# yynil/RWKVTTS

Hardware: AMD Instinct MI355X
Metric: audio-tokens/sec/GPU (train fwd+bwd) RWKV7-0.4B L=4096; 1->8 GPU scaling (higher is better)
Workload: dtype bf16; 1 GPU; RWKV7-0.4B Spark layout train step (fwd+bwd+AdamW), B=8/GPU L=4096, synthetic text+speech tokens, random init (BASELINE.json configs[1]); global_batch=8, seq_len=4096, parallelism=dp1, grad_allreduce=none

## Files before the change

include/rwkv7_hip.h:

```cpp
#ifndef RWKV7_HIP_H
#define RWKV7_HIP_H

#include <stddef.h>

#ifdef __cplusplus
extern "C" {
#endif

#define RWKV7_OK 0
#define RWKV7_EINVAL (-1)
#define RWKV7_ECHUNK (-2)
#define RWKV7_EHEAD  (-3)
#define RWKV7_ESHAPE (-4)

#define RWKV7_HEAD_SIZE 64
#define RWKV7_CHUNK_LEN 16

typedef void *rwkv7_stream_t;

const char *rwkv7_version(void);

int rwkv7_wkv_fwd_bf16(int B, int T, int H, const void *w, const void *q, const void *k, const void *v,
                       const void *a, const void *b, void *y, float *s, float *sa, rwkv7_stream_t stream);
int rwkv7_wkv_fwd_f32(int B, int T, int H, const void *w, const void *q, const void *k, const void *v,
// ... 184 lines not shown
                                   const float *z, const void *e_vk, void *dw, void *dq, void *dk, void *dv,
                                   void *da, void *db, rwkv7_stream_t stream);
int rwkv7_wkv_chunk_fwd_state_bf16(int B, int T, int H, const void *w, const void *q, const void *k, const void *v,
                                   const void *a, const void *b, const float *tinv, void *y, float *sa, void *hs,
                                   const float *h0, float *hT, rwkv7_stream_t stream);
int rwkv7_wkv_chunk_bseq_state_bf16(int B, int T, int H, const void *w, const void *q, const void *a, const void *b,
                                    const void *dy, const float *tinv, void *e_vk, float *z,
                                    const float *dhT, float *dh0, rwkv7_stream_t stream);
int rwkv7_wkv_chunk_fwd_state_seq_bf16(int B, int T, int H, const void *w, const void *q, const void *k, const void *v,
                                       const void *a, const void *b, const float *tinv, void *y, float *sa, void *hs,
                                       const int *seq_chunk_off, int nseq, const float *h0, float *hT, rwkv7_stream_t stream);
int rwkv7_wkv_chunk_bseq_state_seq_bf16(int B, int T, int H, const void *w, const void *q, const void *a, const void *b,
                                        const void *dy, const float *tinv, void *e_vk, float *z, const int *seq_chunk_off, int nseq,
                                        const float *dhT, float *dh0, rwkv7_stream_t stream);
#define RWKV7_STATE_ROW_ZERO (1 << 30)
int rwkv7_wkv_chunk_fwd_state_rows_bf16(int T, int H, const void *w, const void *q, const void *k, const void *v, const void *a,
                                        const void *b, const float *tinv, void *y, const int *seq_chunk_off, int nseq, float *state,
                                        const int *state_row, rwkv7_stream_t stream);
int rwkv7_add_ln_mix_rows_fwd_bf16(int T, int D, int nmix, const void *x, const void *branch, const void *gamma, const void *beta,
                                   float eps, const void *mask, const void *params, const int *prev_src, const int *last_dst,
                                   const void *x_prev_rd, void *x_prev, void *x_out, void *out, int nblocks, int run_len,
                                   rwkv7_stream_t stream);
int rwkv7_cache_rows_commit_bf16(int layers, int n, const void *const *src_tbl, void *const *dst_tbl, const int *src_row,
                                 const int *dst_row, int D, int H, rwkv7_stream_t stream);
#define RWKV7_SEED_ZERO (-1)
int rwkv7_cache_rows_seed_bf16(int layers, int n, const void *const *src_tbl, void *const *dst_tbl, const int *src_row,
                               const int *dst_row, int D, int H, rwkv7_stream_t stream);
int rwkv7_cache_rows_retain_bf16(int layers, int slots, const void *const *src_tbl, void *const *dst_tbl, const unsigned char *live,
                                 unsigned char *armed, const int *retain_row, int *ticket, int D, int H, rwkv7_stream_t stream);
int rwkv7_state_rows_expand_f32(int layers, int n, const void *const *master_tbl, void *const *dst_tbl, const int *voice, int D, int H,
                                rwkv7_stream_t stream);
int rwkv7_state_rows_adamw_f32(int layers, int n, int A, const void *const *grad_tbl, void *const *master_tbl, void *const *m_tbl,
                               void *const *v_tbl, void *const *store_tbl, const int *seg_start, const int *seg_rows, const int *seg_info,
                               const float *skip_flag, float lr, float beta1, float beta2, float eps, float weight_decay,
                               float grad_scale, int D, int H, rwkv7_stream_t stream);
int rwkv7_ce_fwd_bwd_bf16(long rows, int V, void *logits, const long *labels, long ignore_index, float scale, float *loss_rows,
                          rwkv7_stream_t stream);
int rwkv7_ce_fwd_bwd_ls_bf16(long rows, int V, void *logits, const long *labels, long ignore_index, float scale, float *loss_rows,
                             float label_smoothing, rwkv7_stream_t stream);
int rwkv7_ce_fwd_bwd_ld_bf16(long rows, int V, long ld, void *logits, const long *labels, long ignore_index, float scale, float *loss_rows,
                             float label_smoothing, rwkv7_stream_t stream);
int rwkv7_ce_reg_fwd_bwd_bf16(long rows, int V, long ld, void *logits, const long *labels, long ignore_index, float scale, float *loss_rows,
                              float label_smoothing, float z_coef, float max_coef, float *lse_rows, float *max_rows,
                              rwkv7_stream_t stream);
int rwkv7_ce_seq_bwd_bf16(long rows, int V, long ld, void *logits, const long *labels, long ignore_index, long row0, long n_seq,
                          const long *seq_start, const float *seq_scale, float *loss_rows, rwkv7_stream_t stream);
int rwkv7_ce_policy_fwd_bwd_bf16(long rows, int V, long ld, void *logits, const long *labels, long ignore_index, long row0, long n_seq,
                                 const long *seq_start, const float *adv, const float *seq_w, const float *old_lp, const float *ref_lp,
                                 float eps_lo, float eps_hi, float beta, float *lp_rows, float *loss_rows, float *kl_rows,
                                 float *clip_rows, rwkv7_stream_t stream);
int rwkv7_kl_acc_fwd_bwd_bf16(long rows, int V, long ld, const void *logits, void *dlogits, const long *labels, long ignore_index,
                              float smoothing, float scale, float *loss_rows, int *correct_rows, rwkv7_stream_t stream);
int rwkv7_head_eval_bf16(long rows, int V, long ld, const void *logits, const long *labels, long ignore_index, int kind, float smoothing,
                         float *loss_rows, int *correct_rows, int *argmax_rows, rwkv7_stream_t stream);
int rwkv7_seq_scores_f32(long n_seq, const long *seq_start, const float *loss_rows, const int *correct_rows, const long *labels,
                         long ignore_index, double *loss_sum, long *tokens, long *correct, float *worst_loss, long *worst_row,
                         rwkv7_stream_t stream);

int rwkv7_adamw_bf16(long n, float *p32, const void *g16, float *m, float *v, void *p16, float lr, float beta1, float beta2,
                     float eps, float weight_decay, int step, rwkv7_stream_t stream);
int rwkv7_adamw_groups_bf16(long n, float *p32, const void *g16, float *m, float *v, void *p16, const unsigned char *slab_group,
                            const float *group_tab, int ngroups, const float *skip_flag, float lr, float beta1, float beta2,
                            float eps, int step, rwkv7_stream_t stream);
int rwkv7_adamw_groups_clip_bf16(long n, float *p32, const void *g16, float *m, float *v, void *p16, const unsigned char *slab_group,
                                 const float *group_tab, int ngroups, const float *skip_flag, const float *sumsq, float max_norm,
                                 float lr, float beta1, float beta2, float eps, int step, rwkv7_stream_t stream);

long rwkv7_grad_sumsq_workspace_bytes(long n);
int rwkv7_grad_sumsq_bf16(long n, const void *g16, float *partials, float *out, int accumulate, rwkv7_stream_t stream);
int rwkv7_grad_accum_bf16(long n, float *acc32, const void *g16, int first, rwkv7_stream_t stream);
int rwkv7_grad_fold_bf16(long n, const float *acc32, void *g16, float inv_count, rwkv7_stream_t stream);

long rwkv7_buf_digest_workspace_bytes(long n_words);
int rwkv7_buf_digest_u32(long n_words, long first_index, const void *buf, unsigned long long *partials, unsigned long long *out,
                         int accumulate, rwkv7_stream_t stream);
int rwkv7_buf_snapshot_digest_u32(long n_words, long first_index, const void *src, void *dst, unsigned long long *partials,
                                  unsigned long long *out, int accumulate, rwkv7_stream_t stream);

int rwkv7_sum_slabs_bf16(long n, int S, const float *parts, void *out, int accumulate, rwkv7_stream_t stream);
int rwkv7_transpose_bf16(int R, int C, const void *in, void *out, rwkv7_stream_t stream);
int rwkv7_gather_rows_bf16(long n_out, int D, const void *src, const int *idx, void *out, rwkv7_stream_t stream);
int rwkv7_wgrad_skinny_bf16(long M, int N, int K, int S, const void *dy, const void *x, float *parts, rwkv7_stream_t stream);
int rwkv7_wgrad_mid_bf16(long M, int N, int K, int S, const void *dy, const void *x, float *parts, rwkv7_stream_t stream);

int rwkv7_gemm_nt_bf16(int M, int N, int K, const void *A, const void *W, void *C, int epilogue, rwkv7_stream_t stream);
int rwkv7_gemm_nt_relusq_bwd_bf16(int M, int N, int K, const void *A, const void *W, const void *aux, void *C, rwkv7_stream_t stream);
int rwkv7_gemm_nt_relusq_bwd_s_bf16(int M, int N, int K, const void *A, const void *W, const void *s, void *C, rwkv7_stream_t stream);
int rwkv7_gemm_nt_add_bf16(int M, int N, int K, const void *A, const void *W, const void *resid, void *C, rwkv7_stream_t stream);

int rwkv7_mix_lora_wcat_fwd_bf16(int nb, const int *ranks, const void *const *w1, const void *const *mu, int D, void *wcat,
                                 rwkv7_stream_t stream);
int rwkv7_mix_lora_wcat_bwd_bf16(int nb, const int *ranks, const void *const *w1, const void *const *mu, int D, const void *dwcat,
                                 void *const *dw1, void *const *dmu, rwkv7_stream_t stream);
int rwkv7_mix_lora_combine_fwd_bf16(int nb, const int *ranks, const int *acts, long M, int T, const void *G, const void *mask,
                                    void *const *out, rwkv7_stream_t stream);
int rwkv7_mix_lora_combine_bwd_bf16(int nb, const int *ranks, const int *acts, long M, int T, const void *mask, const void *const *y,
                                    const void *const *dy, void *dG, rwkv7_stream_t stream);

int rwkv7_lora_down_pack_bf16(int nb, const int *ranks, const void *const *w1, int D, void *packed, rwkv7_stream_t stream);
int rwkv7_lora_down_fwd_bf16(int nb, const int *ranks, const int *acts, long M, int T, int D, const void *x, const void *mask,
                             const void *const *mu, const void *packed, void *const *out, rwkv7_stream_t stream);

int rwkv7_gemv32_bf16(int M, int N, int K, const void *x, const void *w, const void *bias, void *y, rwkv7_stream_t stream);

enum {
    RWKV7_DEC_LN0_W, RWKV7_DEC_LN0_B, RWKV7_DEC_LN1_W, RWKV7_DEC_LN1_B, RWKV7_DEC_LN2_W, RWKV7_DEC_LN2_B,
    RWKV7_DEC_XR, RWKV7_DEC_XW, RWKV7_DEC_XK, RWKV7_DEC_XV, RWKV7_DEC_XA, RWKV7_DEC_XG,
    RWKV7_DEC_WR, RWKV7_DEC_WK, RWKV7_DEC_WV, RWKV7_DEC_WO,
    RWKV7_DEC_W1, RWKV7_DEC_W2, RWKV7_DEC_W0, RWKV7_DEC_A1, RWKV7_DEC_A2, RWKV7_DEC_A0,
    RWKV7_DEC_V1, RWKV7_DEC_V2, RWKV7_DEC_V0, RWKV7_DEC_G1, RWKV7_DEC_G2,
    RWKV7_DEC_KK, RWKV7_DEC_KA, RWKV7_DEC_RK, RWKV7_DEC_GNW, RWKV7_DEC_GNB,
    RWKV7_DEC_FXK, RWKV7_DEC_WKEY, RWKV7_DEC_WVAL,
    RWKV7_DEC_ATT_XPREV, RWKV7_DEC_ATT_KV , RWKV7_DEC_FFN_XPREV,
    RWKV7_DEC_COUNT
};
typedef struct rwkv7_decode_dims {
    int B, D, H, L, F, V;
    int Rw, Ra, Rv, Rg;
    float ln_eps, gn_eps;
} rwkv7_decode_dims;
int rwkv7_decode_layer_ptrs(void);
size_t rwkv7_decode_workspace_bytes(const rwkv7_decode_dims *dims);
int rwkv7_decode_step_bf16(const rwkv7_decode_dims *dims, const void *const *layer_tbl, const void *x_in, const void *norm_w,
                           const void *norm_b, const void *head_w, const void *head_b, float *logits, void *workspace,
                           int persistent, rwkv7_stream_t stream);
int rwkv7_decode_step_tbl_bf16(const rwkv7_decode_dims *dims, const void *const *layer_tbl, const void *const *layer_tbl_host,
                               const void *x_in, const void *norm_w, const void *norm_b, const void *head_w, const void *head_b,
                               float *logits, void *workspace, int persistent, rwkv7_stream_t stream);
size_t rwkv7_decode_wide_workspace_bytes(const rwkv7_decode_dims *dims);
int rwkv7_decode_step_wide_bf16(const rwkv7_decode_dims *dims, const void *const *layer_tbl, const void *const *layer_tbl_host,
                                const void *x_in, const void *norm_w, const void *norm_b, const void *head_w, const void *head_b,
                                float *logits, void *workspace, rwkv7_stream_t stream);

int rwkv7_sample_rows_f32(int rows, int nseg, const float *logits, long ld, const int *seg_off, const int *seg_len, const int *allow_lo,
                          const int *allow_hi, const int *suppress, int nsuppress, int max_domain, int do_sample, int top_k, float top_p,
                          float temperature, unsigned long long seed, const long *step, long *out, rwkv7_stream_t stream);
typedef struct rwkv7_sample_tail {
    unsigned char *unfinished;
    long eos, pad;
    long *ids;
    long *seq;
    long seq_ld;
    const void *emb;
    void *x;
    int D;
} rwkv7_sample_tail;
int rwkv7_sample_rows_tail_f32(int rows, const float *logits, long ld, const int *seg_off, const int *seg_len, const int *allow_lo,
                               const int *allow_hi, const int *suppress, int nsuppress, int max_domain, int do_sample, int top_k, float top_p,
                               float temperature, unsigned long long seed, const long *step, long *out, const rwkv7_sample_tail *tail,
                               int min_eos_id, long min_eos_until, rwkv7_stream_t stream);
typedef struct rwkv7_slot_state {
    long *step;
    long *limit;
    long *min_until;
    unsigned long long *seed;
    float *inv_temp;
    int *top_k;
    float *top_p;
    unsigned char *do_sample;
    unsigned char *live;
    long *ids;
    long *seq;
    long seq_ld;
    const void *emb;
    void *x;
    int D;
// ... 105 lines not shown
```

rwkvtts_amd/csrc/capi.hip:

```cpp
#include <hip/hip_runtime.h>
#include <math.h>

#include "../../include/rwkv7_hip.h"
#include "launchers.h"
#include "ln_row.h"

using rwkv7::any_null;

extern "C" {

const char *rwkv7_version(void) { return "rwkv7_hip 0.1.0 gfx950"; }

#define FWD_BODY(IMPL, CW)                                                                   \
    if (B <= 0 || T <= 0 || H <= 0 || any_null({w, q, k, v, a, b, y})) return RWKV7_EINVAL; \
    if ((s == nullptr) != (sa == nullptr)) return RWKV7_EINVAL;                              \
    if (T % RWKV7_CHUNK_LEN != 0) return RWKV7_ECHUNK;                                       \
    if ((CW) != 0 && (CW) != 4 && (CW) != 8) return RWKV7_ESHAPE;                            \
    return rwkv7::IMPL(B, T, H, w, q, k, v, a, b, y, s, sa, nullptr, CW, (hipStream_t)stream);

int rwkv7_wkv_fwd_bf16(int B, int T, int H, const void *w, const void *q, const void *k, const void *v,
                       const void *a, const void *b, void *y, float *s, float *sa, rwkv7_stream_t stream) {
    FWD_BODY(wkv_fwd_bf16, 0)
}
int rwkv7_wkv_fwd_f32(int B, int T, int H, const void *w, const void *q, const void *k, const void *v,
// ... 486 lines not shown
    if (rows <= 0 || V <= 0 || any_null({(const void *)logits, (const void *)labels, (const void *)loss_rows})) return RWKV7_EINVAL;
    if (!(label_smoothing >= 0.f && label_smoothing < 1.f)) return RWKV7_EINVAL;
    return rwkv7::ce_fwd_bwd(rows, V, V, logits, labels, ignore_index, scale, loss_rows, label_smoothing, (hipStream_t)stream);
}
int rwkv7_ce_fwd_bwd_ld_bf16(long rows, int V, long ld, void *logits, const long *labels, long ignore_index, float scale, float *loss_rows,
                             float label_smoothing, rwkv7_stream_t stream) {
    if (rows <= 0 || V <= 0 || ld < V || any_null({(const void *)logits, (const void *)labels, (const void *)loss_rows})) return RWKV7_EINVAL;
    if (!(label_smoothing >= 0.f && label_smoothing < 1.f)) return RWKV7_EINVAL;
    return rwkv7::ce_fwd_bwd(rows, V, ld, logits, labels, ignore_index, scale, loss_rows, label_smoothing, (hipStream_t)stream);
}
int rwkv7_ce_reg_fwd_bwd_bf16(long rows, int V, long ld, void *logits, const long *labels, long ignore_index, float scale, float *loss_rows,
                              float label_smoothing, float z_coef, float max_coef, float *lse_rows, float *max_rows,
                              rwkv7_stream_t stream) {
    if (rows <= 0 || V <= 0 || ld < V || any_null({(const void *)logits, (const void *)labels, (const void *)loss_rows})) return RWKV7_EINVAL;
    if (!(label_smoothing >= 0.f && label_smoothing < 1.f)) return RWKV7_EINVAL;
    if (!(z_coef >= 0.f && z_coef < INFINITY && max_coef >= 0.f && max_coef < INFINITY)) return RWKV7_EINVAL;
    return rwkv7::ce_reg_fwd_bwd(rows, V, ld, logits, labels, ignore_index, scale, loss_rows, label_smoothing, z_coef, max_coef, lse_rows,
                                 max_rows, (hipStream_t)stream);
}
int rwkv7_ce_seq_bwd_bf16(long rows, int V, long ld, void *logits, const long *labels, long ignore_index, long row0, long n_seq,
                          const long *seq_start, const float *seq_scale, float *loss_rows, rwkv7_stream_t stream) {
    if (rows <= 0 || V <= 0 || ld < V || row0 < 0 || n_seq <= 0 ||
        any_null({(const void *)logits, (const void *)labels, (const void *)seq_start, (const void *)seq_scale}))
        return RWKV7_EINVAL;
    return rwkv7::ce_seq_bwd(rows, V, ld, logits, labels, ignore_index, row0, n_seq, seq_start, seq_scale, loss_rows, (hipStream_t)stream);
}
int rwkv7_ce_policy_fwd_bwd_bf16(long rows, int V, long ld, void *logits, const long *labels, long ignore_index, long row0, long n_seq,
                                 const long *seq_start, const float *adv, const float *seq_w, const float *old_lp, const float *ref_lp,
                                 float eps_lo, float eps_hi, float beta, float *lp_rows, float *loss_rows, float *kl_rows,
                                 float *clip_rows, rwkv7_stream_t stream) {
    if (rows <= 0 || V <= 0 || ld < V || row0 < 0 || n_seq <= 0 ||
        any_null({(const void *)logits, (const void *)labels, (const void *)seq_start, (const void *)adv, (const void *)seq_w,
                  (const void *)old_lp}))
        return RWKV7_EINVAL;
    if (!(eps_lo >= 0.f && eps_lo < 1.f && eps_hi >= 0.f)) return RWKV7_EINVAL;
    return rwkv7::ce_policy_fwd_bwd(rows, V, ld, logits, labels, ignore_index, row0, n_seq, seq_start, adv, seq_w, old_lp, ref_lp, eps_lo,
                                    eps_hi, beta, lp_rows, loss_rows, kl_rows, clip_rows, (hipStream_t)stream);
}
static float kl_entropy_const(float smoothing, int V) {
    const double s = (double)smoothing;
    return (float)((1.0 - s) * log(1.0 - s) + (s > 0.0 ? s * log(s / (double)(V - 1)) : 0.0));
}
int rwkv7_kl_acc_fwd_bwd_bf16(long rows, int V, long ld, const void *logits, void *dlogits, const long *labels, long ignore_index,
                              float smoothing, float scale, float *loss_rows, int *correct_rows, rwkv7_stream_t stream) {
    if (rows <= 0 || V < 2 || ld < V ||
        any_null({logits, (const void *)dlogits, (const void *)labels, (const void *)loss_rows, (const void *)correct_rows}))
        return RWKV7_EINVAL;
    if (!(smoothing >= 0.f && smoothing < 1.f)) return RWKV7_EINVAL;
    return rwkv7::kl_acc_fwd_bwd(rows, V, ld, logits, dlogits, labels, ignore_index, smoothing, kl_entropy_const(smoothing, V), scale,
                                 loss_rows, correct_rows, (hipStream_t)stream);
}
int rwkv7_head_eval_bf16(long rows, int V, long ld, const void *logits, const long *labels, long ignore_index, int kind, float smoothing,
                         float *loss_rows, int *correct_rows, int *argmax_rows, rwkv7_stream_t stream) {
    if (rows <= 0 || V < 2 || ld < V || (kind != 0 && kind != 1) ||
        any_null({logits, (const void *)labels, (const void *)loss_rows, (const void *)correct_rows}))
        return RWKV7_EINVAL;
    if (!(smoothing >= 0.f && smoothing < 1.f)) return RWKV7_EINVAL;
    const float C = kind == 1 ? kl_entropy_const(smoothing, V) : 0.f;
    return rwkv7::head_eval(rows, V, ld, logits, labels, ignore_index, kind, smoothing, C, loss_rows, correct_rows, argmax_rows,
                            (hipStream_t)stream);
}
int rwkv7_seq_scores_f32(long n_seq, const long *seq_start, const float *loss_rows, const int *correct_rows, const long *labels,
                         long ignore_index, double *loss_sum, long *tokens, long *correct, float *worst_loss, long *worst_row,
                         rwkv7_stream_t stream) {
    if (n_seq <= 0 || n_seq > 0x7fffffffL ||
        any_null({(const void *)seq_start, (const void *)loss_rows, (const void *)correct_rows, (const void *)labels,
                  (const void *)loss_sum, (const void *)tokens, (const void *)correct, (const void *)worst_loss, (const void *)worst_row}))
        return RWKV7_EINVAL;
    return rwkv7::seq_scores(n_seq, seq_start, loss_rows, correct_rows, labels, ignore_index, loss_sum, tokens, correct, worst_loss,
                             worst_row, (hipStream_t)stream);
}
int rwkv7_wgrad_skinny_bf16(long M, int N, int K, int S, const void *dy, const void *x, float *parts, rwkv7_stream_t stream) {
    if (any_null({dy, x, parts})) return RWKV7_EINVAL;
    const int rank = N > K ? K : N, wide = N > K ? N : K;
    if (M <= 0 || S <= 0 || M % S != 0 || (M / S) % 128 != 0 || wide % 256 != 0 || (rank != 32 && rank != 64 && rank != 128))
        return RWKV7_ESHAPE;
    return rwkv7::wgrad_skinny_bf16(M, N, K, S, dy, x, parts, (hipStream_t)stream);
}
int rwkv7_wgrad_mid_bf16(long M, int N, int K, int S, const void *dy, const void *x, float *parts, rwkv7_stream_t stream) {
    if (any_null({dy, x, parts})) return RWKV7_EINVAL;
    if (M <= 0 || S <= 0 || M % S != 0 || (M / S) % 64 != 0 || K <= 0 || K % 256 != 0 || (N != 512 && N != 576)) return RWKV7_ESHAPE;
    return rwkv7::wgrad_mid_bf16(M, N, K, S, dy, x, parts, (hipStream_t)stream);
}
int rwkv7_sum_slabs_bf16(long n, int S, const float *parts, void *out, int accumulate, rwkv7_stream_t stream) {
    if (n <= 0 || S <= 0 || any_null({(const void *)parts, (const void *)out})) return RWKV7_EINVAL;
    if (n % 4 != 0) return RWKV7_ESHAPE;
    return rwkv7::sum_slabs_bf16(n, S, parts, out, accumulate, (hipStream_t)stream);
}
int rwkv7_gather_rows_bf16(long n_out, int D, const void *src, const int *idx, void *out, rwkv7_stream_t stream) {
    if (n_out <= 0 || D <= 0 || any_null({src, (const void *)idx, (const void *)out})) return RWKV7_EINVAL;
    if (D % 8 != 0) return RWKV7_ESHAPE;
    return rwkv7::gather_rows16(n_out, D, src, idx, out, (hipStream_t)stream);
}
int rwkv7_transpose_bf16(int R, int C, const void *in, void *out, rwkv7_stream_t stream) {
    if (R <= 0 || C <= 0 || any_null({in, (const void *)out})) return RWKV7_EINVAL;
    if (R % 64 != 0 || C % 64 != 0) return RWKV7_ESHAPE;
    return rwkv7::transpose_bf16(R, C, in, out, (hipStream_t)stream);
}
int rwkv7_decode_layer_ptrs(void) { return rwkv7::decode_layer_ptrs(); }
size_t rwkv7_decode_workspace_bytes(const rwkv7_decode_dims *dm) {
    if (!dm) return 0;
    return rwkv7::decode_workspace_bytes(dm->B, dm->D, dm->H, dm->F, dm->V, dm->Rw, dm->Ra, dm->Rv, dm->Rg);
}
int rwkv7_decode_step_bf16(const rwkv7_decode_dims *dm, const void *const *layer_tbl, const void *x_in, const void *norm_w,
                           const void *norm_b, const void *head_w, const void *head_b, float *logits, void *workspace,
                           int persistent, rwkv7_stream_t stream) {
    if (!dm || any_null({(const void *)layer_tbl, x_in, norm_w, norm_b, head_w, (const void *)logits, (const void *)workspace}))
        return RWKV7_EINVAL;
    if (dm->H * RWKV7_HEAD_SIZE != dm->D) return RWKV7_EHEAD;
    return rwkv7::decode_step_bf16(dm->B, dm->D, dm->H, dm->L, dm->F, dm->V, dm->Rw, dm->Ra, dm->Rv, dm->Rg, dm->ln_eps, dm->gn_eps,
                                   layer_tbl, nullptr, x_in, norm_w, norm_b, head_w, head_b, logits, workspace, persistent,
                                   (hipStream_t)stream);
}
int rwkv7_decode_step_tbl_bf16(const rwkv7_decode_dims *dm, const void *const *layer_tbl, const void *const *layer_tbl_host,
                               const void *x_in, const void *norm_w, const void *norm_b, const void *head_w, const void *head_b,
                               float *logits, void *workspace, int persistent, rwkv7_stream_t stream) {
    if (!dm || any_null({(const void *)layer_tbl, (const void *)layer_tbl_host, x_in, norm_w, norm_b, head_w, (const void *)logits,
                         (const void *)workspace}))
        return RWKV7_EINVAL;
    if (dm->H * RWKV7_HEAD_SIZE != dm->D) return RWKV7_EHEAD;
    return rwkv7::decode_step_bf16(dm->B, dm->D, dm->H, dm->L, dm->F, dm->V, dm->Rw, dm->Ra, dm->Rv, dm->Rg, dm->ln_eps, dm->gn_eps,
                                   layer_tbl, layer_tbl_host, x_in, norm_w, norm_b, head_w, head_b, logits, workspace, persistent,
                                   (hipStream_t)stream);
}
size_t rwkv7_decode_wide_workspace_bytes(const rwkv7_decode_dims *dm) {
    if (!dm || dm->H * RWKV7_HEAD_SIZE != dm->D) return 0;
    return rwkv7::decode_wide_workspace_bytes(dm->B, dm->D, dm->H, dm->F, dm->V, dm->Rw, dm->Ra, dm->Rv, dm->Rg);
}
int rwkv7_decode_step_wide_bf16(const rwkv7_decode_dims *dm, const void *const *layer_tbl, const void *const *layer_tbl_host,
                                const void *x_in, const void *norm_w, const void *norm_b, const void *head_w, const void *head_b,
                                float *logits, void *workspace, rwkv7_stream_t stream) {
    if (!dm || any_null({(const void *)layer_tbl, x_in, norm_w, norm_b, head_w, (const void *)logits, (const void *)workspace}))
        return RWKV7_EINVAL;
    if (dm->H * RWKV7_HEAD_SIZE != dm->D) return RWKV7_EHEAD;
    return rwkv7::decode_step_wide_bf16(dm->B, dm->D, dm->H, dm->L, dm->F, dm->V, dm->Rw, dm->Ra, dm->Rv, dm->Rg, dm->ln_eps, dm->gn_eps,
                                        layer_tbl, layer_tbl_host, x_in, norm_w, norm_b, head_w, head_b, logits, workspace,
                                        (hipStream_t)stream);
}
int rwkv7_sample_rows_f32(int rows, int nseg, const float *logits, long ld, const int *seg_off, const int *seg_len, const int *allow_lo,
                          const int *allow_hi, const int *suppress, int nsuppress, int max_domain, int do_sample, int top_k, float top_p,
                          float temperature, unsigned long long seed, const long *step, long *out, rwkv7_stream_t stream) {
    if (rows <= 0 || nseg <= 0 || max_domain <= 0 || nsuppress < 0 ||
        any_null({(const void *)logits, (const void *)seg_off, (const void *)seg_len, (const void *)step, (const void *)out}) ||
        (nsuppress > 0 && !suppress))
        return RWKV7_EINVAL;
    return rwkv7::sample_rows_f32(rows, nseg, logits, ld, seg_off, seg_len, allow_lo, allow_hi, suppress, nsuppress, max_domain, do_sample,
                                  top_k, top_p, temperature, seed, step, out, nullptr, -1, 0, (hipStream_t)stream);
}
int rwkv7_sample_rows_tail_f32(int rows, const float *logits, long ld, const int *seg_off, const int *seg_len, const int *allow_lo,
                               const int *allow_hi, const int *suppress, int nsuppress, int max_domain, int do_sample, int top_k, float top_p,
                               float temperature, unsigned long long seed, const long *step, long *out, const rwkv7_sample_tail *tail,
                               int min_eos_id, long min_eos_until, rwkv7_stream_t stream) {
    if (rows <= 0 || max_domain <= 0 || nsuppress < 0 ||
        any_null({(const void *)logits, (const void *)seg_off, (const void *)seg_len, (const void *)step, (const void *)out}) ||
        (nsuppress > 0 && !suppress))
        return RWKV7_EINVAL;
    return rwkv7::sample_rows_f32(rows, 1, logits, ld, seg_off, seg_len, allow_lo, allow_hi, suppress, nsuppress, max_domain, do_sample, top_k,
                                  top_p, temperature, seed, step, out, tail, min_eos_id, min_eos_until, (hipStream_t)stream);
}
static bool sample_slots_args_ok(int rows, const float *logits, const int *allow_lo, const int *allow_hi, const int *suppress, int nsuppress,
                                 int max_domain, const rwkv7_slot_state *st) {
    if (rows <= 0 || !st || !logits || max_domain <= 0 || nsuppress < 0 || (nsuppress > 0 && !suppress) || (!allow_lo != !allow_hi))
        return false;
    return !(any_null({(const void *)st->step, (const void *)st->limit, (const void *)st->min_until, (const void *)st->seed,
                       (const void *)st->inv_temp, (const void *)st->top_k, (const void *)st->top_p, (const void *)st->do_sample,
                       (const void *)st->live, (const void *)st->ids, (const void *)st->seq}) ||
// ... 106 lines not shown
```

rwkvtts_amd/csrc/launchers.h:

```cpp
#pragma once
#include <hip/hip_runtime.h>
#include <stddef.h>
#include <stdint.h>

#include <initializer_list>

namespace rwkv7 {

inline bool any_null(std::initializer_list<const void *> ps) {
    for (const void *p : ps)
        if (!p) return true;
    return false;
}

int wkv_fwd_bf16(int B, int T, int H, const void *w, const void *q, const void *k, const void *v, const void *a, const void *b, void *y,
                 float *s, float *sa, float *state, int force_cw, hipStream_t stream);
int wkv_fwd_f32(int B, int T, int H, const void *w, const void *q, const void *k, const void *v, const void *a, const void *b, void *y,
                float *s, float *sa, float *state, int force_cw, hipStream_t stream);
int wkv_bwd_bf16(int B, int T, int H, const void *w, const void *q, const void *k, const void *v, const void *a, const void *b,
                 const void *dy, const float *s, const float *sa, void *dw, void *dq, void *dk, void *dv, void *da, void *db,
                 hipStream_t stream);
int wkv_bwd_f32(int B, int T, int H, const void *w, const void *q, const void *k, const void *v, const void *a, const void *b,
                const void *dy, const float *s, const float *sa, void *dw, void *dq, void *dk, void *dv, void *da, void *db,
                hipStream_t stream);
int wkv_bwd_split_bf16(int B, int T, int H, const void *w, const void *q, const void *k, const void *v, const void *a, const void *b,
                       const void *dy, const float *s, const float *sa, void *const *dw, void *const *dq, void *const *dk, void *dv,
                       void *const *da, void *const *db, int wide, hipStream_t stream);
int wkv_bwd_split_f32(int B, int T, int H, const void *w, const void *q, const void *k, const void *v, const void *a, const void *b,
                      const void *dy, const float *s, const float *sa, void *const *dw, void *const *dq, void *const *dk, void *dv,
                      void *const *da, void *const *db, int wide, hipStream_t stream);

int chunk_prep_bf16(int B, int T, int H, const void *w, const void *a, const void *b, float *tinv, hipStream_t stream);
int chunk_prep_f32(int B, int T, int H, const void *w, const void *a, const void *b, float *tinv, hipStream_t stream);
int chunk_fwd_bf16(int B, int T, int H, const void *w, const void *q, const void *k, const void *v, const void *a, const void *b,
                   const float *tinv, void *y, float *sa, void *hs, const int *seq_chunk_off, int nseq, hipStream_t stream);
int chunk_fwd_f32(int B, int T, int H, const void *w, const void *q, const void *k, const void *v, const void *a, const void *b,
                  const float *tinv, void *y, float *sa, void *hs, const int *seq_chunk_off, int nseq, hipStream_t stream);
int chunk_fwd9_state_seq_bf16(int B, int T, int H, const void *w, const void *q, const void *k, const void *v, const void *a,
                              const void *b, const float *tinv, void *y, float *sa, void *hs, const int *seq_chunk_off, int nseq,
                              const float *h0, float *hT, hipStream_t stream);
int chunk_fwd9_state_rows_bf16(int T, int H, const void *w, const void *q, const void *k, const void *v, const void *a, const void *b,
                               const float *tinv, void *y, const int *seq_chunk_off, int nseq, float *state, const int *state_row,
                               hipStream_t stream);
int chunk_bseq_bf16(int B, int T, int H, const void *w, const void *q, const void *a, const void *b, const void *dy, const float *tinv,
                    void *e_vk, float *z, const int *seq_chunk_off, int nseq, hipStream_t stream);
int chunk_bseq_state_seq_bf16(int B, int T, int H, const void *w, const void *q, const void *a, const void *b, const void *dy,
                              const float *tinv, void *e_vk, float *z, const int *seq_chunk_off, int nseq, const float *dhT, float *dh0,
                              hipStream_t stream);
int chunk_bwd_out10_bf16(int B, int T, int H, const void *w, const void *q, const void *k, const void *v, const void *a, const void *b,
                         const void *dy, const void *hs, const float *sa, const float *z, const void *e_vk, void *dw, void *dq, void *dk,
                         void *dv, void *da, void *db, hipStream_t stream);
int chunk_debug_mma(const float *X, const float *Y, float *D, float *DT, hipStream_t stream);
int chunk_debug_tr16(const uint16_t *in, const int *addr, uint16_t *out, hipStream_t stream);

int gemm_nt4_bf16(int M, int N, int K, const void *A, const void *W, void *C, const void *aux, int epilogue, hipStream_t stream);
int gemv32_bf16(int M, int N, int K, const void *x, const void *w, const void *bias, void *y, hipStream_t stream);
int lora32_bf16(int M, int N, int K, int R, int act, const void *x, const void *w1, const void *w2, const void *bias, void *y,
                hipStream_t stream);
int wgrad_skinny_bf16(long M, int N, int K, int S, const void *dy, const void *x, float *parts, hipStream_t stream);
int wgrad_mid_bf16(long M, int N, int K, int S, const void *dy, const void *x, float *parts, hipStream_t stream);

struct MixLoraDesc {
    int nb;
    int r[4], off[4];
    int act[4];
    const void *w1[4];
    const void *mu[4];
    void *out[4];
    void *out2[4];
};
int mix_lora_wcat_fwd(const MixLoraDesc &d, int R, int D, void *wcat, hipStream_t stream);
int mix_lora_wcat_bwd(const MixLoraDesc &d, int R, int D, const void *dwcat, hipStream_t stream);
int mix_lora_combine_fwd(const MixLoraDesc &d, long M, int T, int R, const void *G, const void *mask, hipStream_t stream);
int mix_lora_combine_bwd(const MixLoraDesc &d, long M, int T, int R, const void *mask, void *dG, hipStream_t stream);

struct LoraDownDesc {
    int nb;
    int r[4], off[4];
    int act[4];
    const void *w1[4];
    const void *mu[4];
    void *out[4];
    int tile0[5];
};
int lora_down_pack(const LoraDownDesc &d, int R, int D, void *packed, hipStream_t stream);
int lora_down_fwd(LoraDownDesc &d, int R, long M, int T, int D, const void *x, const void *mask, const void *packed, hipStream_t stream);

int sum_slabs_bf16(long n, int S, const float *parts, void *out, int accumulate, hipStream_t stream);
int transpose_bf16(int R, int C, const void *in, void *out, hipStream_t stream);
int gather_rows16(long n_out, int D, const void *src, const int *idx, void *out, hipStream_t stream);

int add_ln_mix_rows_fwd_bf16(int T, int D, int nmix, const void *x, const void *branch, const void *gamma, const void *beta, float eps,
                             const void *mask, const void *params, const int *prev_src, const int *last_dst, const void *x_prev_rd,
                             void *x_prev, void *x_out, void *out, int nblocks, int run_len, hipStream_t stream);
int cache_rows_commit_bf16(int layers, int n, const void *const *src_tbl, void *const *dst_tbl, const int *src_row, const int *dst_row,
                           int D, int H, hipStream_t stream);
int cache_rows_seed_bf16(int layers, int n, const void *const *src_tbl, void *const *dst_tbl, const int *src_row, const int *dst_row,
                         int D, int H, hipStream_t stream);
int cache_rows_retain_bf16(int layers, int slots, const void *const *src_tbl, void *const *dst_tbl, const unsigned char *live,
                           unsigned char *armed, const int *retain_row, int *ticket, int D, int H, hipStream_t stream);

int state_rows_expand_f32(int layers, int n, const void *const *master_tbl, void *const *dst_tbl, const int *voice, int D, int H,
                          hipStream_t stream);
int state_rows_adamw_f32(int layers, int A, const void *const *grad_tbl, void *const *master_tbl, void *const *m_tbl, void *const *v_tbl,
                         void *const *store_tbl, const int *seg_start, const int *seg_rows, const int *seg_info, const float *skip_flag,
                         float lr, float beta1, float beta2, float eps, float wd, float grad_scale, int D, int H, hipStream_t stream);

int ce_fwd_bwd(long rows, int V, long ld, void *logits, const long *labels, long ignore_index, float scale, float *loss_rows,
               float label_smoothing, hipStream_t stream);
int ce_reg_fwd_bwd(long rows, int V, long ld, void *logits, const long *labels, long ignore_index, float scale, float *loss_rows,
                   float label_smoothing, float z_coef, float max_coef, float *lse_rows, float *max_rows, hipStream_t stream);
int ce_seq_bwd(long rows, int V, long ld, void *logits, const long *labels, long ignore_index, long row0, long n_seq,
               const long *seq_start, const float *seq_scale, float *loss_rows, hipStream_t stream);
int ce_policy_fwd_bwd(long rows, int V, long ld, void *logits, const long *labels, long ignore_index, long row0, long n_seq,
                      const long *seq_start, const float *adv, const float *seq_w, const float *old_lp, const float *ref_lp, float eps_lo,
                      float eps_hi, float beta, float *lp_rows, float *loss_rows, float *kl_rows, float *clip_rows, hipStream_t stream);
int kl_acc_fwd_bwd(long rows, int V, long ld, const void *logits, void *dlogits, const long *labels, long ignore_index, float smoothing,
                   float C, float scale, float *loss_rows, int *correct_rows, hipStream_t stream);
int head_eval(long rows, int V, long ld, const void *logits, const long *labels, long ignore_index, int kind, float smoothing, float C,
              float *loss_rows, int *correct_rows, int *argmax_rows, hipStream_t stream);
int seq_scores(long n_seq, const long *seq_start, const float *loss_rows, const int *correct_rows, const long *labels, long ignore_index,
               double *loss_sum, long *tokens, long *correct, float *worst_loss, long *worst_row, hipStream_t stream);

int adamw_step(long n, float *p32, const void *g16, float *m, float *v, void *p16, const uint8_t *slab_group, const float *group_tab,
               const float *skip_flag, float lr, float beta1, float beta2, float eps, float wd, float inv_bc1, float inv_sqrt_bc2,
               hipStream_t stream);
int adamw_clip_step(long n, float *p32, const void *g16, float *m, float *v, void *p16, const uint8_t *slab_group, const float *group_tab,
                    const float *skip_flag, const float *sumsq, float max_norm, float lr, float beta1, float beta2, float eps, float wd,
                    float inv_bc1, float inv_sqrt_bc2, hipStream_t stream);
int grad_sumsq_bf16(long n, const void *g16, float *partials, float *out, int accumulate, hipStream_t stream);
int grad_accum_bf16(long n, float *acc32, const void *g16, int first, hipStream_t stream);
int grad_fold_bf16(long n, const float *acc32, void *g16, float inv_count, hipStream_t stream);
long buf_digest_tiles(long n_words);
int buf_digest_u32(long n_words, long first_index, const void *buf, void *dst, unsigned long long *partials, unsigned long long *out,
                   int accumulate, hipStream_t stream);

int sample_rows_f32(int rows, int nseg, const float *logits, long ld, const int *seg_off, const int *seg_len, const int *allow_lo,
                    const int *allow_hi, const int *suppress, int nsuppress, int max_domain, int do_sample, int top_k, float top_p,
                    float temperature, unsigned long long seed, const long *step, long *out, const void *tail, int min_id, long min_until,
                    hipStream_t stream);
int sample_slots_f32(int rows, const float *logits, long ld, const int *row_slot, const int *allow_lo, const int *allow_hi,
                     const int *suppress, int nsuppress, int max_domain, const void *st, hipStream_t stream);
int sample_slots_lp_f32(int rows, const float *logits, long ld, const int *row_slot, const int *allow_lo, const int *allow_hi,
// ... 41 lines not shown
```

rwkvtts_amd/fused.py:

```python
import ctypes
import os

import torch

from . import _lib

_FWD_BLOCKS = 32768
_MIX_FWD_BLOCKS = 2048
_BWD_BLOCKS = 1024
_MIX_BWD_ROWS = 4
_MIX_BWD_BLOCKS = 1024


def _sfx(t):
    if not t.is_cuda:
        raise NotImplementedError("fused RWKV-7 stages run on the HIP device only (no CPU path)")
    if t.dtype == torch.bfloat16:
        return "bf16"
    if t.dtype == torch.float32:
        return "f32"
    raise TypeError(f"bf16 or fp32 expected, got {t.dtype}")


def _c(t):
# ... 571 lines not shown
        dout = _c(dout)
        compact = COMPACT_POST_BWD
        if compact:
            part_post = torch.empty(nb, 3, D, dtype=torch.float32, device=k.device)
            d_y, dt_post, d_g = [torch.empty_like(k) for _ in range(3)]
            hscal = torch.empty(rows, H, 2, dtype=torch.float32, device=k.device)
            d_r_post = d_k2_post = d_v2_post = None
            _call("tmix_post_bwd_compact", k, rows, D, dout, y, r, k2, v2, g, gn_w, gn_b, r_k, ctx.eps, d_y, dt_post, d_g, hscal, part_post,
                  nb)
        else:
            (d_y, d_r_post, d_k2_post, d_v2_post, d_g), part_post = _tmix_post_bwd(dout, y, r, k2, v2, g, gn_w, gn_b, r_k, ctx.eps)
        if WGRAD_SYNC_BEFORE_SCAN:
            wgrad_side_sync(k.device)
        v4 = lambda t: t.view(B, T, H, 64)
        if ctx.chunked_fwd:
            dw, dq, dk, dv, da, db = ops.wkv7_chunk_backward(v4(w), v4(r), v4(k2), v4(v2), v4(a_in), v4(b_in), v4(d_y), s, sa,
                                                             tinv, seq_off=ctx.seq_start)
            dw2, dq2, dk2, da2, db2 = [(g, None) for g in (dw, dq, dk, da, db)]
        elif ctx.via_op:
            dw, dq, dk, dv, da, db = [torch.empty_like(k).view(B, T, H, 64) for _ in range(6)]
            torch.ops.wind_backstepping.backward(v4(w), v4(r), v4(k2), v4(v2), v4(a_in), v4(b_in), v4(d_y), s, sa, dw, dq, dk, dv, da, db)
            dw2, dq2, dk2, da2, db2 = [(g, None) for g in (dw, dq, dk, da, db)]
        else:
            dw2, dq2, dk2, dv, da2, db2 = ops.wkv7_backward_split(v4(w), v4(r), v4(k2), v4(v2), v4(a_in), v4(b_in),
                                                                  v4(d_y), s, sa)
        d_wpre, d_k, d_v, d_apre, d_r = [torch.empty_like(k) for _ in range(5)]
        d_vpre = torch.empty_like(k) if v_pre is not None else None
        d_vf = torch.empty_like(k) if v_pre is not None else None
        part = torch.empty(nb, 5, D, dtype=torch.float32, device=k.device)
        d_vf_next = None if (d_vf_next is None or v_pre is None) else _c(d_vf_next)
        gsum = [dw2[0], dw2[1], dk2[0], dk2[1], d_k2_post, dv, d_v2_post, da2[0], da2[1], db2[0], db2[1],
                dq2[0], dq2[1], d_r_post, d_vf_next]
        if compact:
            gsum += [dt_post, r, r_k, hscal]
        ptrs = _lib.ptr_array(gsum)
        _call("tmix_prepare_bwd_sum_compact" if compact else "tmix_prepare_bwd_sum", k, rows, D, w_pre, k, v, a_pre, v_pre, v_first, mask,
              k_k, k_a, ptrs, d_wpre, d_k, d_v, d_apre, d_vpre, d_vf, d_r, part, nb)
        dp = _colsum(part, k.dtype)
        dpp = _colsum(part_post, k.dtype)
        _attach_colsums(dp, d_wpre, d_apre, d_vpre)
        return (d_r, d_wpre, d_k, d_v, d_apre, d_g, d_vpre, d_vf, dp[0], dp[1], dpp[0], dpp[1], dpp[2], None, None,
                None, None)


def tmix_core(r, w_pre, k, v, a_pre, g, v_pre, v_first, k_k, k_a, gn_weight, gn_bias, r_k, mask, H, eps, is_layer0,
              seq_start=None):
    assert k.shape[-1] == H * 64
    if is_layer0:
        v_pre = v_first = None
    res = _TmixCore.apply(r, w_pre, k, v, a_pre, g, v_pre, v_first, k_k, k_a, gn_weight, gn_bias, r_k.reshape(-1),
                          _mask_rows(mask, k), H, eps, seq_start)
    if torch.is_tensor(res):
        return res, None
    return res


def lora_decode_supported(x, rank):
    rows = x.numel() // x.shape[-1]
    return (GEMV_MAX_ROWS and x.is_cuda and x.dtype == torch.bfloat16 and rows <= GEMV_MAX_ROWS and rank in (32, 64, 128)
            and x.shape[-1] % 64 == 0 and not torch.is_grad_enabled())


def lora_decode(x, w1, w2, bias, activation):
    K, N, R = x.shape[-1], w2.shape[0], w1.shape[0]
    rows = x.numel() // K
    x2 = _c(x).view(rows, K)
    b2 = None if bias is None else _c(bias)
    y = torch.empty(rows, N, dtype=torch.bfloat16, device=x.device)
    _lib.call("rwkv7_lora32_bf16", x, rows, N, K, R, _ACT_CODE[activation], x2, _c(w1), _c(w2), b2, y)
    return y.view(*x.shape[:-1], N)


WGRAD_MIN_ROWS = 4096
WGRAD_SLABS_SMALL, WGRAD_SLABS_BIG = 8, 4
COMPACT_POST_BWD = True
SKINNY_WGRAD = True


MID_WGRAD = os.environ.get("RWKV7_MID_WGRAD", "1") == "1"
MID_WGRAD_SLABS = 32
MID_WGRAD_HITS = [0]


def wgrad_splitk(dy2, x2, out=None, slabs=None):
    M, N = dy2.shape
    K = x2.shape[1]
    rank, wide = min(N, K), max(N, K)
    if (SKINNY_WGRAD and dy2.dtype == torch.bfloat16 and x2.dtype == torch.bfloat16 and rank in (32, 64, 128) and wide % 256 == 0
            and M >= WGRAD_MIN_ROWS and M % 512 == 0):
        S = M // 512
        part = torch.empty(S, N, K, dtype=torch.float32, device=dy2.device)
        if out is None:
            out = torch.empty(N, K, dtype=torch.bfloat16, device=dy2.device)
        _lib.call("rwkv7_wgrad_skinny_bf16", part, M, N, K, S, dy2, x2, part)
        _lib.call("rwkv7_sum_slabs_bf16", part, N * K, S, part, out, 0)
        return out
    if (MID_WGRAD and dy2.dtype == torch.bfloat16 and x2.dtype == torch.bfloat16 and N in (512, 576) and K % 256 == 0 and M >= WGRAD_MIN_ROWS
            and M % (MID_WGRAD_SLABS * 64) == 0 and dy2.is_contiguous() and x2.is_contiguous()):
        S = MID_WGRAD_SLABS
        part = torch.empty(S, N, K, dtype=torch.float32, device=dy2.device)
        if out is None:
            out = torch.empty(N, K, dtype=torch.bfloat16, device=dy2.device)
        _lib.call("rwkv7_wgrad_mid_bf16", part, M, N, K, S, dy2, x2, part)
        _lib.call("rwkv7_sum_slabs_bf16", part, N * K, S, part, out, 0)
        MID_WGRAD_HITS[0] += 1
        return out
    S = slabs if slabs else (WGRAD_SLABS_SMALL if N * K <= 1024 * 1024 else WGRAD_SLABS_BIG)
    if M < WGRAD_MIN_ROWS or M % (S * 8) != 0:
        res = torch.mm(dy2.t(), x2)
        if out is not None:
            out.copy_(res)
            return out
        return res
    part = torch.bmm(dy2.view(S, M // S, N).transpose(1, 2), x2.view(S, M // S, K), out_dtype=torch.float32)
    if dy2.dtype != torch.bfloat16 or (N * K) % 4 != 0:
        res = part.sum(0).to(dy2.dtype)
        if out is not None:
            out.copy_(res)
            return out
        return res
    if out is None:
        out = torch.empty(N, K, dtype=torch.bfloat16, device=dy2.device)
    _lib.call("rwkv7_sum_slabs_bf16", part, N * K, S, part, out, 0)
    return out


GATHER_ROWS_KERNEL = os.environ.get("RWKV7_GATHER_ROWS_KERNEL", "1") == "1"


class _GatherRows(torch.autograd.Function):

    @staticmethod
    def forward(ctx, src, idx, inv):
        src = _c(src)
        out = torch.empty(idx.numel(), src.shape[1], dtype=src.dtype, device=src.device)
        _lib.call("rwkv7_gather_rows_bf16", src, idx.numel(), src.shape[1], src, idx, out)
        ctx.save_for_backward(idx, inv)
        return out

    @staticmethod
    def backward(ctx, g):
        idx, inv = ctx.saved_tensors
        g = _c(g)
        dsrc = torch.empty(inv.numel(), g.shape[1], dtype=g.dtype, device=g.device)
        _lib.call("rwkv7_gather_rows_bf16", g, inv.numel(), g.shape[1], g, inv, dsrc)
        return dsrc, None, None


def gather_rows(src, idx, inv):
    if (GATHER_ROWS_KERNEL and src.is_cuda and src.dtype == torch.bfloat16 and src.shape[1] % 8 == 0 and idx.dtype == torch.int32
            and inv.dtype == torch.int32):
        return _GatherRows.apply(src, idx, inv)
    out = src.index_select(0, idx.clamp(min=0).long())
    return out * (idx >= 0).unsqueeze(-1).to(out.dtype)


WGRAD_SIDE_STREAM = os.environ.get("RWKV7_WGRAD_SIDE_STREAM", "0") == "1"
WGRAD_SYNC_BEFORE_SCAN = False
_SIDE = {}


def wgrad_side_sync(device=None):
    for idx, ent in _SIDE.items():
        if ent[1] and (device is None or device.index == idx):
            torch.cuda.current_stream(ent[0].device).wait_stream(ent[0])
            ent[1] = False


def _wgrad(d2, x2, param):
    slot = _grad_slot(param)
    if slot is None:
        wgrad_side_sync(d2.device)
        return wgrad_splitk(d2, x2)
    if not WGRAD_SIDE_STREAM:
        wgrad_splitk(d2, x2, out=slot)
        return slot.view_as(param)
    ent = _SIDE.get(d2.device.index)
    if ent is None:
        ent = _SIDE[d2.device.index] = [torch.cuda.Stream(d2.device), False]
# ... 317 lines not shown
```

Baseline: 272,100 tokens/s.

## Add split-K TN MFMA weight-gradient kernel for FFN-shaped layers

Adds a custom HIP weight-gradient kernel that computes dy^T·x for the 4096x1024 and 1024x4096 FFN shapes. It uses 256x256 tiles, double-buffered LDS staging with register prefetch, and scheduled 32x32x16 bf16 MFMAs. Results are split over 4 row slabs into fp32 partials, which are then reduced to bf16. The goal is to replace the torch bmm split-K path for these large weight gradients, at the cost of extra fp32 partial buffer traffic and a separate reduction pass.

```diff
diff --git a/include/rwkv7_hip.h b/include/rwkv7_hip.h
--- a/include/rwkv7_hip.h
+++ b/include/rwkv7_hip.h
@@ -290,6 +290,7 @@
 int rwkv7_gather_rows_bf16(long n_out, int D, const void *src, const int *idx, void *out, rwkv7_stream_t stream);
 int rwkv7_wgrad_skinny_bf16(long M, int N, int K, int S, const void *dy, const void *x, float *parts, rwkv7_stream_t stream);
 int rwkv7_wgrad_mid_bf16(long M, int N, int K, int S, const void *dy, const void *x, float *parts, rwkv7_stream_t stream);
+int rwkv7_wgrad_tn_bf16(long M, int N, int K, int S, const void *dy, const void *x, float *parts, rwkv7_stream_t stream);
 
 int rwkv7_gemm_nt_bf16(int M, int N, int K, const void *A, const void *W, void *C, int epilogue, rwkv7_stream_t stream);
 int rwkv7_gemm_nt_relusq_bwd_bf16(int M, int N, int K, const void *A, const void *W, const void *aux, void *C, rwkv7_stream_t stream);
diff --git a/rwkvtts_amd/csrc/capi.hip b/rwkvtts_amd/csrc/capi.hip
--- a/rwkvtts_amd/csrc/capi.hip
+++ b/rwkvtts_amd/csrc/capi.hip
@@ -592,6 +592,12 @@
     if (M <= 0 || S <= 0 || M % S != 0 || (M / S) % 64 != 0 || K <= 0 || K % 256 != 0 || (N != 512 && N != 576)) return RWKV7_ESHAPE;
     return rwkv7::wgrad_mid_bf16(M, N, K, S, dy, x, parts, (hipStream_t)stream);
 }
+int rwkv7_wgrad_tn_bf16(long M, int N, int K, int S, const void *dy, const void *x, float *parts, rwkv7_stream_t stream) {
+    if (any_null({dy, x, parts})) return RWKV7_EINVAL;
+    if (M <= 0 || S <= 0 || N <= 0 || K <= 0) return RWKV7_EINVAL;
+    if (M % S != 0 || M / S > 0x7fffffffL || (M / S) % 128 != 0 || N % 256 != 0 || K % 256 != 0) return RWKV7_ESHAPE;
+    return rwkv7::wgrad_tn_bf16(M, N, K, S, dy, x, parts, (hipStream_t)stream);
+}
 int rwkv7_sum_slabs_bf16(long n, int S, const float *parts, void *out, int accumulate, rwkv7_stream_t stream) {
     if (n <= 0 || S <= 0 || any_null({(const void *)parts, (const void *)out})) return RWKV7_EINVAL;
     if (n % 4 != 0) return RWKV7_ESHAPE;
diff --git a/rwkvtts_amd/csrc/launchers.h b/rwkvtts_amd/csrc/launchers.h
--- a/rwkvtts_amd/csrc/launchers.h
+++ b/rwkvtts_amd/csrc/launchers.h
@@ -59,6 +59,7 @@
                 hipStream_t stream);
 int wgrad_skinny_bf16(long M, int N, int K, int S, const void *dy, const void *x, float *parts, hipStream_t stream);
 int wgrad_mid_bf16(long M, int N, int K, int S, const void *dy, const void *x, float *parts, hipStream_t stream);
+int wgrad_tn_bf16(long M, int N, int K, int S, const void *dy, const void *x, float *parts, hipStream_t stream);
 
 struct MixLoraDesc {
     int nb;
diff --git a/rwkvtts_amd/csrc/wgrad_tn.hip b/rwkvtts_amd/csrc/wgrad_tn.hip
--- /dev/null
+++ b/rwkvtts_amd/csrc/wgrad_tn.hip
@@ -0,0 +1,134 @@
+#include "launchers.h"
+#include "chunk_common.h"
+#include "launch_attr.h"
+
+namespace rwkv7 {
+
+namespace {
+constexpr int kTnTile = 256;
+constexpr int kTnStep = 32;
+constexpr int kTnLd = kTnTile + 32;
+constexpr int kTnPF = 4;
+constexpr int kTnPlane = kTnStep * kTnLd;
+constexpr size_t kTnLds = 4 * kTnPlane * sizeof(uint16_t);
+
+__global__ __launch_bounds__(256) void wgrad_tn_kernel(int N, int K, int rows_per_slab, const bf16_t *__restrict__ dy_, const bf16_t *__restrict__ x_,
+                                                       float *__restrict__ part) {
+    extern __shared__ __attribute__((aligned(16))) uint16_t s_tn[];
+    const int tid = threadIdx.x, lane = tid & 63;
+    const int wave = __builtin_amdgcn_readfirstlane(tid >> 6), wm = wave >> 1, wn = wave & 1;
+    const int ntk = K / kTnTile, tiles = (N / kTnTile) * ntk;
+    int lin = blockIdx.x;
+    if ((gridDim.x & 7) == 0) lin = (blockIdx.x & 7) * (gridDim.x >> 3) + (blockIdx.x >> 3);
+    const int slab = lin / tiles, tile = lin - slab * tiles;
+    const int n0 = (tile / ntk) * kTnTile, k0 = (tile % ntk) * kTnTile;
+    const long row0 = (long)slab * rows_per_slab;
+    const uint16_t *ga = reinterpret_cast<const uint16_t *>(dy_) + row0 * N + n0;
+    const uint16_t *gb = reinterpret_cast<const uint16_t *>(x_) + row0 * K + k0;
+    const int crow = tid >> 5, ccol = (tid & 31) * 8;
+    const int nsteps = rows_per_slab / kTnStep;
+    struct Regs { uint4 a0, a1, a2, a3, b0, b1, b2, b3; };
+    auto fetch = [&](int step) {
+        Regs r;
+        step = step < nsteps ? step : nsteps - 1;
+        const uint16_t *a = ga + ((long)step * kTnStep + crow) * N + ccol, *b = gb + ((long)step * kTnStep + crow) * K + ccol;
+        r.a0 = *reinterpret_cast<const uint4 *>(a);
+        r.a1 = *reinterpret_cast<const uint4 *>(a + 8L * N);
+        r.a2 = *reinterpret_cast<const uint4 *>(a + 16L * N);
+        r.a3 = *reinterpret_cast<const uint4 *>(a + 24L * N);
+        r.b0 = *reinterpret_cast<const uint4 *>(b);
+        r.b1 = *reinterpret_cast<const uint4 *>(b + 8L * K);
+        r.b2 = *reinterpret_cast<const uint4 *>(b + 16L * K);
+        r.b3 = *reinterpret_cast<const uint4 *>(b + 24L * K);
+        return r;
+    };
+    auto stage = [&](int buf, const Regs r) {
+        uint16_t *sa = s_tn + buf * 2 * kTnPlane + crow * kTnLd + ccol, *sb = sa + kTnPlane;
+        *reinterpret_cast<uint4 *>(sa) = r.a0;
+        *reinterpret_cast<uint4 *>(sa + 8 * kTnLd) = r.a1;
+        *reinterpret_cast<uint4 *>(sa + 16 * kTnLd) = r.a2;
+        *reinterpret_cast<uint4 *>(sa + 24 * kTnLd) = r.a3;
+        *reinterpret_cast<uint4 *>(sb) = r.b0;
+        *reinterpret_cast<uint4 *>(sb + 8 * kTnLd) = r.b1;
+        *reinterpret_cast<uint4 *>(sb + 16 * kTnLd) = r.b2;
+        *reinterpret_cast<uint4 *>(sb + 24 * kTnLd) = r.b3;
+    };
+    f32x16 acc[4][4];
+#pragma unroll
+    for (int i = 0; i < 4; i++)
+#pragma unroll
+        for (int j = 0; j < 4; j++) acc[i][j] = zero16();
+    struct Frags { bf16x8 a[4], b[4]; };
+    auto read_frags = [&](Frags &F, int buf, int ks) {
+        const uint16_t *sa = s_tn + buf * 2 * kTnPlane, *sb = sa + kTnPlane;
+#pragma unroll
+        for (int i = 0; i < 4; i++) F.a[i] = frag_tr(sa, kTnLd, 16 * ks, wm * 128 + i * 32, lane);
+#pragma unroll
+        for (int j = 0; j < 4; j++) F.b[j] = frag_tr(sb, kTnLd, 16 * ks, wn * 128 + j * 32, lane);
+    };
+    auto mfma16 = [&](const Frags &F) {
+#pragma unroll
+        for (int i = 0; i < 4; i++)
+#pragma unroll
+            for (int j = 0; j < 4; j++) acc[i][j] = __builtin_amdgcn_mfma_f32_32x32x16_bf16(F.a[i], F.b[j], acc[i][j], 0, 0, 0);
+    };
+    Regs r0 = fetch(0), r1 = fetch(1), r2 = fetch(2), r3 = fetch(3);
+    stage(0, r0);
+    r0 = fetch(kTnPF);
+    lds_barrier();
+    Frags F0, F1;
+    read_frags(F0, 0, 0);
+#define WGT_STEP(R_, U_)                                                                                                  \
+    read_frags(F1, (U_) & 1, 1);                                                                                          \
+    stage(((U_) + 1) & 1, R_);                                                                                            \
+    mfma16(F0);                                                                                                           \
+    _Pragma("unroll") for (int q = 0; q < 8; q++) {                                         \
+        __builtin_amdgcn_sched_group_barrier(0x008, 1, 0);                                                                \
+        __builtin_amdgcn_sched_group_barrier(0x100, 2, 0);                                                                \
+    }                                                                                                                     \
+    _Pragma("unroll") for (int q = 0; q < 8; q++) {                                            \
+        __builtin_amdgcn_sched_group_barrier(0x008, 1, 0);                                                                \
+        __builtin_amdgcn_sched_group_barrier(0x200, 1, 0);                                                                \
+    }                                                                                                                     \
+    lds_barrier();                                                                                                        \
+    __builtin_amdgcn_sched_barrier(0);                                                                                    \
+    R_ = fetch(step + (U_) + 1 + kTnPF);                                                                                  \
+    read_frags(F0, ((U_) + 1) & 1, 0);                                                                                    \
+    mfma16(F1);                                                                                                           \
+    _Pragma("unroll") for (int q = 0; q < 8; q++) {                                 \
+        __builtin_amdgcn_sched_group_barrier(0x008, 1, 0);                                                                \
+        __builtin_amdgcn_sched_group_barrier(0x020, 1, 0);                                                                \
+        __builtin_amdgcn_sched_group_barrier(0x100, 2, 0);                                                                \
+    }                                                                                                                     \
+    __builtin_amdgcn_sched_group_barrier(0x008, 8, 0);                                                                    \
+    __builtin_amdgcn_sched_barrier(0);
+    for (int step = 0; step < nsteps; step += kTnPF) {
+        WGT_STEP(r1, 0)
+        WGT_STEP(r2, 1)
+        WGT_STEP(r3, 2)
+        WGT_STEP(r0, 3)
+    }
+#undef WGT_STEP
+    float *p = part + (long)slab * N * K;
+#pragma unroll
+    for (int i = 0; i < 4; i++)
+#pragma unroll
+        for (int j = 0; j < 4; j++) {
+            const int nb = n0 + wm * 128 + i * 32, kb = k0 + wn * 128 + j * 32;
+#pragma unroll
+            for (int r = 0; r < 16; r++) p[(long)(nb + d_row(r, lane)) * K + kb + (lane & 31)] = acc[i][j][r];
+        }
+}
+}
+
+int wgrad_tn_bf16(long M, int N, int K, int S, const void *dy, const void *x, float *part, hipStream_t st) {
+    static DynLdsOnce lds_once;
+    if (N % kTnTile || K % kTnTile || M % S || (M / S) % (kTnStep * kTnPF)) return -4;
+    if (hipError_t e = lds_once.ensure(reinterpret_cast<const void *>(&wgrad_tn_kernel), (int)kTnLds); e != hipSuccess) return (int)e;
+    (void)hipGetLastError();
+    const int grid = (N / kTnTile) * (K / kTnTile) * S;
+    wgrad_tn_kernel<<<dim3(grid), dim3(256), kTnLds, st>>>(N, K, (int)(M / S), (const bf16_t *)dy, (const bf16_t *)x, part);
+    return (int)hipGetLastError();
+}
+
+}
diff --git a/rwkvtts_amd/fused.py b/rwkvtts_amd/fused.py
--- a/rwkvtts_amd/fused.py
+++ b/rwkvtts_amd/fused.py
@@ -677,6 +677,26 @@
 MID_WGRAD_HITS = [0]
 
 
+TN_WGRAD = os.environ.get("RWKV7_TN_WGRAD", "1") == "1"
+TN_WGRAD_CLASSES = {(4096, 1024): 4, (1024, 4096): 4}
+TN_WGRAD_HITS = [0]
+
+
+def _wgrad_tn(dy2, x2, out, S):
+    M, N = dy2.shape
+    K = x2.shape[1]
+    part = torch.empty(S, N, K, dtype=torch.float32, device=dy2.device)
+    try:
+        _lib.call("rwkv7_wgrad_tn_bf16", part, M, N, K, S, dy2, x2, part)
+    except ValueError:
+        return None
+    if out is None:
+        out = torch.empty(N, K, dtype=torch.bfloat16, device=dy2.device)
+    _lib.call("rwkv7_sum_slabs_bf16", part, N * K, S, part, out, 0)
+    TN_WGRAD_HITS[0] += 1
+    return out
+
+
 def wgrad_splitk(dy2, x2, out=None, slabs=None):
     M, N = dy2.shape
     K = x2.shape[1]
@@ -690,6 +710,11 @@
         _lib.call("rwkv7_wgrad_skinny_bf16", part, M, N, K, S, dy2, x2, part)
         _lib.call("rwkv7_sum_slabs_bf16", part, N * K, S, part, out, 0)
         return out
+    if (TN_WGRAD and (N, K) in TN_WGRAD_CLASSES and dy2.dtype == torch.bfloat16 and x2.dtype == torch.bfloat16 and M >= WGRAD_MIN_ROWS
+            and dy2.is_contiguous() and x2.is_contiguous()):
+        res = _wgrad_tn(dy2, x2, out, slabs if slabs else TN_WGRAD_CLASSES[(N, K)])
+        if res is not None:
+            return res
     if (MID_WGRAD and dy2.dtype == torch.bfloat16 and x2.dtype == torch.bfloat16 and N in (512, 576) and K % 256 == 0 and M >= WGRAD_MIN_ROWS
             and M % (MID_WGRAD_SLABS * 64) == 0 and dy2.is_contiguous() and x2.is_contiguous()):
         S = MID_WGRAD_SLABS
```

New measurement: 275,100 tokens/s (median of 6 runs). 1.1% higher.
